# ndpp/ndpp

Hardware: AMD Instinct MI355X
Metric: E_in points*Legendre-orders/sec (free-gas scatter moments) (higher is better)
Workload: dtype f64

## Files before the change

### ndpp_amd/csrc/fg_pipeline.h

```cpp
#pragma once

#include "ndpp_math.h"

namespace ndpp {
#if NDPP_FAST
inline namespace fast_arith {
#else
inline namespace strict_arith {
#endif

#if NDPP_FAST
constexpr int kMuBlock = 2;
#else
constexpr int kMuBlock = 1;
#endif
constexpr int kSegPerGroup = 5;
constexpr int kMaxLevels = 32;
constexpr int kStackLdsLevels = 8;
constexpr int kMaxRows = 2;
constexpr int kSplitLog2 = 4;
constexpr int kSplit = 1 << kSplitLog2;
constexpr int kRowBits = 16;

enum { kStatKEvals = 0, kStatMuVisits, kStatMuIntegrals, kStatEoutNodes,
       kStatWaveIters, kStatLaneIters, kStatOrderVisits, kStatGaussIntegrals, kNumStats };

NDPP_HD unsigned chan_bit(int r, int l) { return 1u << (r * kRowBits + l); }

struct FgBatch {
  int n_jobs, R, G, L, M;
  double A, kT;
  const double* job_A = nullptr;
  const double* job_kT = nullptr;
  const double* job_ein;
  const int* job_row;
  const double* f_tab;
  const double* e_bins;
  double sab_threshold, brent_thresh, mu_tol, eout_tol;
  int mu_its, eout_its;
  MuGrid grid;
  int ncap;
  double* node_a;
  double* node_b;
  double* node_F;
  double* node_S;
  int* node_info;
  int tcap;
  double* t_mulo;
  double* t_muhi;
  double* t_X;
  unsigned char* t_gl = nullptr;
  double gl_ratio = 2.0;
  int gl_near = 1;
  double gl_amin = 2.0E-6;
  int gl_cert_depth = 7;
  int gl_cert_depth_near = 8;
  int gl_panels = 16;
  int gl_graded = 8;
  int* lvl_cnt;
  int* next_task;
  int* overflow;
  unsigned long long* stats;
  double* seg = nullptr;
  int split_below = 0;
  const int* order = nullptr;
  const int* mask_rank = nullptr;
  const int* mu_nodes = nullptr;
  double* raw;

  NDPP_HD double A_of(int job) const { return job_A ? job_A[job] : A; }
  NDPP_HD double kT_of(int job) const { return job_kT ? job_kT[job] : kT; }
  NDPP_HD int nch() const { return R * L; }
  NDPP_HD int n_trees() const { return n_jobs * G * kSegPerGroup; }
  NDPP_HD int lvl_off(int level) const {
    int o = 0;
    for (int k = 0; k < level; ++k) o += lvl_cnt[k];
    return o;
  }
  NDPP_HD bool split_level(int level) const {
    const int nt = n_mu_tasks(level);
    return seg != nullptr && nt > 0 && nt <= split_below;
  }
  NDPP_HD int tasks_per_node(int level) const { return level == 0 ? 5 : 2; }
  NDPP_HD int n_tasks(int level) const { return lvl_cnt[level] * tasks_per_node(level); }
  NDPP_HD int n_mu_tasks(int level) const {
    return (mu_nodes ? *mu_nodes : lvl_cnt[level]) * tasks_per_node(level);
  }
  NDPP_HD int rec_index(int level, int base, int n, int slot) const {
    return level == 0 ? 5 * n + slot : 2 * (n - base) + (slot == 3 ? 1 : 0);
  }
  NDPP_HD double& F(int slot, int ch, int n) const {
    return node_F[((size_t)(slot * R * L + ch)) * ncap + n];
  }
  NDPP_HD double& S(int ch, int n) const { return node_S[(size_t)ch * ncap + n]; }
  NDPP_HD double& tX(int k, int r, int t) const { return t_X[((size_t)(k * R + r)) * tcap + t]; }
  NDPP_HD unsigned full_mask() const {
    unsigned m = 0;
    for (int r = 0; r < R; ++r) m |= ((1u << L) - 1u) << (r * kRowBits);
    return m;
  }
  NDPP_HD int node_job(int n) const { return node_info[4 * n + 2] & 0x3ffffff; }
  NDPP_HD int node_depth(int n) const { return node_info[4 * n + 2] >> 26; }
};

NDPP_HD void fg_setup_group(const FgBatch& B, int job, int g) {
  const double Ein = B.job_ein[job];
  const double A = B.A_of(job), kT = B.kT_of(job);
  double alphaEin = (A - 1.0) / (A + 1.0);
  alphaEin = alphaEin * alphaEin * Ein;
  double Eout_lo, Eout_hi;
  fg_eout_bounds(A, kT, Ein, Eout_lo, Eout_hi);
  const double eg = B.e_bins[g], eg1 = B.e_bins[g + 1];

  double sa[kSegPerGroup], sb[kSegPerGroup];
  bool on[kSegPerGroup] = {false, false, false, false, false};
  if ((eg < Eout_hi) && (eg1 > Eout_lo)) {
    double Elo = (Eout_lo > eg) ? Eout_lo : eg;
    double Ehi = (Eout_hi < eg1) ? Eout_hi : eg1;
    double Ebottom = (eg == 0.0) ? 0.01 * Elo : eg;
    sa[0] = Ebottom; sb[0] = Elo; on[0] = true;
    sa[1] = Ehi;     sb[1] = eg1; on[1] = true;
    if ((Elo < alphaEin) && (alphaEin < Ehi)) {
      sa[2] = Elo; sb[2] = alphaEin; on[2] = true;
      Elo = alphaEin;
    }
    if ((Elo < Ein) && (Ein < Ehi)) {
      sa[3] = Elo; sb[3] = Ein; on[3] = true;
      Elo = Ein;
    }
    sa[4] = Elo; sb[4] = Ehi; on[4] = true;
  } else {
    sa[4] = eg; sb[4] = eg1; on[4] = true;
  }
  const unsigned full = B.full_mask();
  const int nch = B.nch();
  for (int s = 0; s < kSegPerGroup; ++s) {
    int n = (job * B.G + g) * kSegPerGroup + s;
    bool live = on[s] && (sa[s] != sb[s]);
    B.node_a[n] = live ? sa[s] : 0.0;
    B.node_b[n] = live ? sb[s] : 0.0;
    B.node_info[4 * n + 0] = live ? (int)full : 0;
    B.node_info[4 * n + 1] = -1;
    B.node_info[4 * n + 2] = job;
    B.node_info[4 * n + 3] = 0;
    for (int ch = 0; ch < nch; ++ch) B.S(ch, n) = 0.0;
  }
}

NDPP_HD void fg_task_decode(const FgBatch& B, int level, int base, int t, int& n,
                            int& slot) {
  (void)B;
  int idx;
  if (level == 0) {
    idx = t / 5;
    slot = t - 5 * idx;
  } else {
    idx = t >> 1;
    slot = 1 + 2 * (t & 1);
  }
  n = B.order ? B.order[idx] : (level == 0 ? idx : base + idx);
}

NDPP_HD unsigned fg_sort_key(const FgBatch& B, unsigned mask) {
  unsigned m = 0;
  for (int r = 0; r < B.R; ++r) m |= (mask >> (r * kRowBits)) & ((1u << B.L) - 1u);
  return m;
}

constexpr int kSortClasses = 4;
NDPP_HD int fg_node_bucket(const FgBatch& B, int level, int base, int n, int nb) {
  const unsigned mask = (unsigned)B.node_info[4 * n + 0];
  const int last = kSortClasses * nb - 1;
  if (mask == 0) return last;
  double wmax = -1.0;
  const int nslots = B.tasks_per_node(level);
  for (int k = 0; k < nslots; ++k) {
    const int slot = level == 0 ? k : 1 + 2 * k;
    const int rec = B.rec_index(level, base, n, slot);
    unsigned m = mask;
    if (B.t_gl) {
      const unsigned rows = B.t_gl[rec];
      for (int r = 0; r < B.R; ++r)
        if (rows >> r & 1u) m &= ~(((1u << kRowBits) - 1u) << (r * kRowBits));
    }
    if (m == 0) continue;
    const double km = fmax(fmax(fabs(B.tX(0, 0, rec)), fabs(B.tX(1, 0, rec))), fabs(B.tX(2, 0, rec)));
    const double w = (B.t_muhi[rec] - B.t_mulo[rec]) * km;
    wmax = fmax(wmax, w >= 0.0 ? w : 0.0);
  }
  if (wmax < 0.0) return last;
  const int cls = wmax >= 1073741824.0 ? 0 : wmax >= 1048576.0 ? 1 : wmax >= 256.0 ? 2 : 3;
  int b = cls * nb + B.mask_rank[fg_sort_key(B, mask)];
  return b < last ? b : last - 1;
}

NDPP_HD double fg_slot_point(double a, double b, int slot) {
  double c = 0.5 * (a + b);
  switch (slot) {
    case 0: return a;
    case 1: return 0.5 * (a + c);
    case 2: return c;
    case 3: return 0.5 * (c + b);
    default: return b;
  }
}

template <int R>
NDPP_HD void fg_Krows(const FgPair& q, const MuGrid& g, const double* const* f, double mu,
                      double* K) {
#if NDPP_FAST
  const double E = fg_E(q, mu);
#pragma unroll
  for (int r = 0; r < R; ++r) K[r] = (q.C1 * fg_fval(g, f[r], mu)) * E;
#else
  fg_K_rows<R>(q, g, f, mu, K);
#endif
}
NDPP_HD double simpson(double w, double f0, double f1, double f2) {
  return w * (fma(4.0, f1, f0) + f2);
}

NDPP_HD bool fg_gauss_box(int mu_its, double mu_tol) {
  return mu_its >= 15 && mu_tol <= 1.0E-7;
}
constexpr unsigned kGaussNear = 0x80u;
NDPP_HD unsigned fg_gauss_zone(const FgBatch& B, const FgPair& q, double Ein, double Eout) {
  const double amin = (q.EpE - 2.0 * q.s2) / q.AkT;
  if (!(amin >= B.gl_amin)) return 0u;
  const unsigned rows = (1u << B.R) - 1u;
  if (Eout >= B.gl_ratio * Ein || Ein >= B.gl_ratio * Eout) return rows;
  return B.gl_near ? (rows | kGaussNear) : 0u;
}

NDPP_HD void fg_prep_task(const FgBatch& B, int level, int base, int t) {
  int n, slot;
  if (level == 0) { n = t / 5; slot = t - 5 * n; }
  else { n = base + (t >> 1); slot = 1 + 2 * (t & 1); }
  if (B.node_info[4 * n + 0] == 0) {
    if (B.t_gl) B.t_gl[t] = 0;
    return;
  }
  const int job = B.node_job(n);
  const double Ein = B.job_ein[job];
  const double Eout = fg_slot_point(B.node_a[n], B.node_b[n], slot);
  const double A = B.A_of(job);
  const FgPair q = make_pair(A, B.kT_of(job), Ein, Eout);
  double mlo, mhi;
  fg_find_mu(q, A, Ein, Eout, B.sab_threshold, B.brent_thresh, mlo, mhi);
  const double mc = (mlo + mhi) * 0.5;
  B.t_mulo[t] = mlo;
  B.t_muhi[t] = mhi;
  if (B.t_gl) B.t_gl[t] = (unsigned char)fg_gauss_zone(B, q, Ein, Eout);
  for (int r = 0; r < B.R; ++r) {
    const double* fr[1] = {B.f_tab + (size_t)B.job_row[(size_t)job * B.R + r] * B.M};
    fg_Krows<1>(q, B.grid, fr, mlo, &B.tX(0, r, t));
    fg_Krows<1>(q, B.grid, fr, mhi, &B.tX(1, r, t));
    fg_Krows<1>(q, B.grid, fr, mc, &B.tX(2, r, t));
  }
}

#if NDPP_FAST
constexpr int kGaussN = 16;
NDPP_HD double gauss_node(int j) {
  constexpr double x[kGaussN] = {
      -0.98940093499164994, -0.9445750230732326, -0.86563120238783176, -0.755404408355003,
      -0.61787624440264377, -0.45801677765722737, -0.28160355077925892, -0.095012509837637454,
      0.095012509837637454, 0.28160355077925892, 0.45801677765722737, 0.61787624440264377,
      0.755404408355003, 0.86563120238783176, 0.9445750230732326, 0.98940093499164994};
  return x[j];
}
NDPP_HD double gauss_weight(int j) {
  constexpr double w[kGaussN] = {
      0.027152459411754037, 0.062253523938647706, 0.095158511682492591, 0.12462897125553403,
      0.14959598881657676, 0.16915651939500262, 0.18260341504492361, 0.18945061045506859,
      0.18945061045506859, 0.18260341504492361, 0.16915651939500262, 0.14959598881657676,
      0.12462897125553403, 0.095158511682492591, 0.062253523938647706, 0.027152459411754037};
  return w[j];
}

template <int R, int LMAX, bool kAdd = false>
NDPP_HD void gauss_composite(const FgBatch& B, const FgPair& q, const FView<R>& fv, double a, double b,
                             int panels, const PnConsts& pk, double* acc) {
  if (!kAdd) {
#pragma unroll
    for (int ch = 0; ch < R * LMAX; ++ch) acc[ch] = 0.0;
  }
  const double h = (b - a) / (double)(2 * panels);
  for (int p = 0; p < panels; ++p) {
    const double c = a + h * (double)(2 * p + 1);
    for (int j = 0; j < kGaussN; j += 2) {
      const double mu0 = fma(h, gauss_node(j), c), mu1 = fma(h, gauss_node(j + 1), c);
      FvLoad v0[R], v1[R];
      fg_fval_load_rows<R>(B.grid, fv, mu0, v0);
      fg_fval_load_rows<R>(B.grid, fv, mu1, v1);
      double E0, E1;
      fg_E2(q, mu0, mu1, E0, E1);
      E0 *= h * gauss_weight(j);
      E1 *= h * gauss_weight(j + 1);
      double P0[LMAX], P1[LMAX];
      pn_all<LMAX>(mu0, P0, pk);
      pn_all<LMAX>(mu1, P1, pk);
#pragma unroll
      for (int r = 0; r < R; ++r) {
        const double K0 = (q.C1 * fg_fval_use(v0[r])) * E0;
        const double K1 = (q.C1 * fg_fval_use(v1[r])) * E1;
#pragma unroll
        for (int l = 0; l < LMAX; ++l) acc[r * LMAX + l] = fma(K1, P1[l], fma(K0, P0[l], acc[r * LMAX + l]));
      }
    }
  }
}

template <int R, int LMAX>
NDPP_HD void gauss_graded(const FgBatch& B, const FgPair& q, const FView<R>& fv, double a, double b,
                          int m, int split, const PnConsts& pk, double* acc) {
#pragma unroll
  for (int ch = 0; ch < R * LMAX; ++ch) acc[ch] = 0.0;
  const double W = b - a;
  double lo = a;
  for (int k = 1; k <= m + 1; ++k) {
    const double hi = k <= m ? b - ldexp(W, -k) : b;
    gauss_composite<R, LMAX, true>(B, q, fv, lo, hi, split, pk, acc);
// ... 38 lines not shown
    for (int j = 0; j < nn; ++j) {
      const double xa = a + hd * (double)j;
      const double xb = (j == nn - 1) ? b : a + hd * (double)(j + 1);
      const double xc = 0.5 * (xa + xb), xd = 0.5 * (xa + xc), xe = 0.5 * (xc + xb);
      double Kd[R], Ke[R], Kc[R], Kb[R];
      Kat(xd, xe, Kd, Ke);
      if (dep == 0) {
#pragma unroll
        for (int r = 0; r < R; ++r) { Kc[r] = B.tX(2, r, t); Kb[r] = B.tX(1, r, t); }
        evals += 2;
      } else {
        Kat(xc, xb, Kc, Kb);
        if (j == nn - 1) {
#pragma unroll
          for (int r = 0; r < R; ++r) Kb[r] = B.tX(1, r, t);
        }
        evals += 4;
      }
      double Pd[LMAX], Pc[LMAX], Pe[LMAX], Pb[LMAX];
      pn_all<LMAX>(xd, Pd, pk); pn_all<LMAX>(xc, Pc, pk); pn_all<LMAX>(xe, Pe, pk); pn_all<LMAX>(xb, Pb, pk);
      unsigned leaf = 0, big = 0;
#pragma unroll
      for (int r = 0; r < R; ++r) {
        const double Xc2 = 2.0 * Kc[r], Xc4 = 4.0 * Kc[r], Kd4 = 4.0 * Kd[r], Ke4 = 4.0 * Ke[r];
#pragma unroll
        for (int l = 0; l < LMAX; ++l) {
          const double T = fma(Kb[r], Pb[l], Ka[r] * Pa[l]);
          const double s1 = fma(Xc4, Pc[l], T);
          const double s2 = fma(Ke4, Pe[l], fma(Kd4, Pd[l], fma(Xc2, Pc[l], T)));
          const double dS = fabs(fma(w, s2, -(wp * s1)));
          if (mask & chan_bit(r, l)) {
            if (!(dS > eps15)) leaf |= chan_bit(r, l);
            if (dS > big15) big |= chan_bit(r, l);
          }
        }
      }
      const unsigned bad = strict ? leaf : ((leaf & prev_big) | (prev_leaf & big));
#pragma unroll
      for (int r = 0; r < R; ++r)
        if (bad & (((1u << kRowBits) - 1u) << (r * kRowBits))) rows &= ~(1u << r);
      if (rows == 0) return 0;
      prev_leaf = leaf;
      prev_big = big;
#pragma unroll
      for (int r = 0; r < R; ++r) Ka[r] = Kb[r];
#pragma unroll
      for (int l = 0; l < LMAX; ++l) Pa[l] = Pb[l];
    }
  }
  return rows;
}

constexpr int kGaussCertPhases = 2;
constexpr int kGaussPhGraded = kGaussCertPhases;
constexpr int kGaussPhLadder = kGaussCertPhases + 1;
constexpr int kGaussPhases = kGaussCertPhases + 2;
NDPP_HD int gauss_cert_split(int p) {
  return p == 0 ? 0 : p == 1 ? kCertDepth : kMaxLevels;
}

constexpr int kGaussDone = 2;
static_assert(kMaxRows <= kGaussDone, "rows in play and rows done share one byte with kGaussNear");
struct GaussCand {
  int t;
  unsigned st;
};

NDPP_HD int gauss_cert_depth(const FgBatch& B, unsigned st) {
  return (st & kGaussNear) ? B.gl_cert_depth_near : B.gl_cert_depth;
}
NDPP_HD bool gauss_phase_on(const FgBatch& B, int p, unsigned st) {
  if (p < kGaussCertPhases) return gauss_cert_split(p) < gauss_cert_depth(B, st);
  if (p == kGaussPhGraded) return (st & kGaussNear) && B.gl_graded > 0;
  return p == kGaussPhLadder;
}
NDPP_HD int gauss_next_phase(const FgBatch& B, int p, unsigned st) {
  do ++p; while (p < kGaussPhases && !gauss_phase_on(B, p, st));
  return p;
}

template <int R>
NDPP_HD unsigned mu_gauss_entry(const FgBatch& B, int level, int base, int t) {
  unsigned rows = B.t_gl[t];
  if (!rows) return 0;
  const unsigned near = rows & kGaussNear;
  rows &= ~kGaussNear;
  const int n_node = level == 0 ? t / 5 : base + (t >> 1);
  const unsigned mask = (unsigned)B.node_info[4 * n_node + 0];
#pragma unroll
  for (int r = 0; r < R; ++r)
    if (!(mask & (((1u << kRowBits) - 1u) << (r * kRowBits)))) rows &= ~(1u << r);
  if (rows == 0) { B.t_gl[t] = 0; return 0; }
  return rows | near;
}

template <int R, int LMAX>
NDPP_HD int mu_gauss_phase(const FgBatch& B, int level, int base, int p, GaussCand& c, int& next) {
  const int t = c.t;
  const unsigned near = c.st & kGaussNear;
  unsigned rows = c.st & ((1u << R) - 1u);
  unsigned done = (c.st >> kGaussDone) & ((1u << R) - 1u);
  int n_node, slot;
  if (level == 0) { n_node = t / 5; slot = t - 5 * n_node; }
  else { n_node = base + (t >> 1); slot = 1 + 2 * (t & 1); }
  const unsigned mask = (unsigned)B.node_info[4 * n_node + 0];
  const int job = B.node_job(n_node);
  const double Ein = B.job_ein[job];
  const double Eout = fg_slot_point(B.node_a[n_node], B.node_b[n_node], slot);
  const FgPair q = make_pair(B.A_of(job), B.kT_of(job), Ein, Eout);
  FRows f;
  f.off = 8u * (unsigned)B.M * (unsigned)B.job_row[(size_t)job * R];
  const FView<R> fv = f_view<R>(B.f_tab, f, B.M);
  const double a = B.t_mulo[t], b = B.t_muhi[t];
  const PnConsts pk = make_pn_consts();
  int evals = 0;
  auto finish = [&](unsigned taken) {
    B.t_gl[t] = (unsigned char)taken;
    next = kGaussPhases;
  };
  if (p < kGaussCertPhases) {
    const int cd = gauss_cert_depth(B, c.st);
    const int hi = gauss_cert_split(p + 1) < cd ? gauss_cert_split(p + 1) : cd;
    rows = mu_gauss_certify<R, LMAX>(B, q, fv, t, mask, rows, gauss_cert_split(p), hi, pk, evals);
    if (rows == 0) { finish(0u); return evals; }
    c.st = near | rows;
    next = gauss_next_phase(B, p, c.st);
    return evals;
  }
  double Ic[R * LMAX], If[R * LMAX];
  auto take_agreeing_rows = [&]() {
#pragma unroll
    for (int r = 0; r < R; ++r) {
      if (!((rows & ~done) >> r & 1u)) continue;
      bool ok = true;
#pragma unroll
      for (int l = 0; l < LMAX; ++l)
        ok = ok && (fabs(If[r * LMAX + l] - Ic[r * LMAX + l]) <= kGaussAgree * fabs(If[r * LMAX]));
      if (!ok) continue;
      done |= 1u << r;
#pragma unroll
      for (int l = 0; l < LMAX; ++l)
        if (l < B.L && (mask & chan_bit(r, l))) B.F(slot, r * B.L + l, n_node) = If[r * LMAX + l];
    }
  };
  if (p == kGaussPhGraded) {
    gauss_graded<R, LMAX>(B, q, fv, a, b, B.gl_graded, 1, pk, Ic);
    gauss_graded<R, LMAX>(B, q, fv, a, b, B.gl_graded, 2, pk, If);
    evals += 3 * (B.gl_graded + 1) * kGaussN;
    take_agreeing_rows();
    if (done == rows) { finish(rows); return evals; }
    c.st = near | rows | (done << kGaussDone);
    next = kGaussPhLadder;
    return evals;
  }
  gauss_composite<R, LMAX>(B, q, fv, a, b, 4, pk, Ic);
  evals += 4 * kGaussN;
  for (int n = 8;; n *= 2) {
    gauss_composite<R, LMAX>(B, q, fv, a, b, n, pk, If);
    evals += n * kGaussN;
    take_agreeing_rows();
    if (done == rows || 2 * n > B.gl_panels) break;
#pragma unroll
    for (int k = 0; k < R * LMAX; ++k) Ic[k] = If[k];
  }
  finish(done);
  return evals;
}
// ... 321 lines not shown
#pragma unroll
    for (int r = 0; r < R; ++r) { s.Xb[r] = Xbj[r]; s.Xc[r] = Xej[r]; }
    s.wp = wj;
    s.mask = mj;
    s.depth = dj + 1;
    return true;
  }
  return false;
}

template <int R, int LMAX>
NDPP_HD void mu_finish(const FgBatch& B, const MuLane<R, LMAX>& s, bool split = false) {
  const unsigned mask = s.chans;
#pragma unroll
  for (int r = 0; r < R; ++r)
#pragma unroll
    for (int l = 0; l < LMAX; ++l)
      if (mask & chan_bit(r, l)) {
        if (split) {
          if (!s.own_pending)
            B.seg[((size_t)s.task * kSplit + s.slot_path) * B.nch() + r * B.L + l] = s.acc[r * LMAX + l];
          continue;
        }
        B.F(s.slot, r * B.L + l, s.node) = s.tot[r * LMAX + l] + s.acc[r * LMAX + l];
      }
}

template <int R, int LMAX>
NDPP_HD void mu_init_split(const FgBatch& B, int level, int base, int t, MuLane<R, LMAX>& s) {
  const int nt = B.n_mu_tasks(level);
  const int i = t % nt, rank = t / nt;
  mu_init<R, LMAX>(B, level, base, i, s);
  int jp = 0;
  if (s.mask != 0) {
#if NDPP_FAST
    const double pa = s.q.p, qa = s.q.q;
#else
    const double pa = s.q.EpE / s.q.AkT, qa = 2.0 * s.q.s2 / s.q.AkT;
#endif
    const double x = ((pa - fabs(s.q.beta)) / qa - s.a) / (s.b - s.a) * (double)kSplit;
    jp = (x > 0.0) ? (x < (double)(kSplit - 1) ? (int)x : kSplit - 1) : 0;
  }
  int lo = jp - 1, hi = jp, cur = hi;
  for (int k = 0; k <= rank; ++k) {
    if (((k & 1) == 0 && hi < kSplit) || lo < 0) cur = hi++;
    else cur = lo--;
  }
  s.path_left = kSplitLog2;
  s.path_bits = (unsigned)cur;
  s.slot_path = 0;
  int tz = 0;
  while (tz < kSplitLog2 && !(((unsigned)cur >> tz) & 1u)) ++tz;
  s.own_from = kSplitLog2 - tz;
  s.own_pending = (s.own_from != 0);
}

NDPP_HD void fg_mu_combine_task(const FgBatch& B, int level, int base, int t) {
  int n, slot;
  fg_task_decode(B, level, base, t, n, slot);
  const unsigned mask = (unsigned)B.node_info[4 * n + 0];
  if (mask == 0) return;
  const unsigned gl_rows = B.t_gl ? B.t_gl[B.rec_index(level, base, n, slot)] : 0u;
  const int nch = B.nch();
  for (int r = 0; r < B.R; ++r)
    for (int l = 0; l < B.L; ++l)
      if ((mask & chan_bit(r, l)) && !(gl_rows >> r & 1u)) {
        const int ch = r * B.L + l;
        double tot = 0.0;
        for (int j = 0; j < kSplit; ++j) tot = tot + B.seg[((size_t)t * kSplit + j) * nch + ch];
        B.F(slot, ch, n) = tot;
      }
}

struct HostAtomics {
  static int add(int* p, int v) { int o = *p; *p += v; return o; }
};

template <class Atomics>
NDPP_HD void fg_node_process(const FgBatch& B, int level, int base, int i) {
  const int n = base + i;
  const unsigned mask = (unsigned)B.node_info[4 * n + 0];
  if (mask == 0) return;
  const int depth = B.node_depth(n);
  const double a = B.node_a[n], b = B.node_b[n];
  const double c = 0.5 * (a + b);
  const double h = b - a;
  const double w = h / 12.0;
  const double eps15 = 15.0 * ldexp(B.eout_tol, -depth);
  const bool bottom = (B.eout_its - depth) <= 0;
  unsigned refine = 0;
  auto half = [w](double f0, double f1, double f2) { return w * (f0 + 4.0 * f1 + f2); };
  for (int r = 0; r < B.R; ++r)
    for (int l = 0; l < B.L; ++l) {
      if (!(mask & chan_bit(r, l))) continue;
      const int ch = r * B.L + l;
      const double Fa = B.F(0, ch, n), Fd = B.F(1, ch, n), Fc = B.F(2, ch, n),
                   Fe = B.F(3, ch, n), Fb = B.F(4, ch, n);
      double S = B.S(ch, n);
      if (depth == 0) S = (h / 6.0) * (Fa + 4.0 * Fc + Fb);
      const double S2 = half(Fa, Fd, Fc) + half(Fc, Fe, Fb);
      if (bottom || (fabs(S2 - S) <= eps15)) {
        B.S(ch, n) = S2 + (S2 - S) / 15.0;
      } else {
        refine |= chan_bit(r, l);
      }
    }
  B.node_info[4 * n + 3] = (int)refine;
  if (!refine) return;
  const int pos = Atomics::add(&B.lvl_cnt[level + 1], 2);
  const int left = base + B.lvl_cnt[level] + pos;
  if (left + 2 > B.ncap) {
    *B.overflow = 1;
    B.node_info[4 * n + 3] = 0;
    return;
  }
  B.node_info[4 * n + 1] = left;
  const int job = B.node_job(n);
  for (int k = 0; k < 2; ++k) {
    const int m = left + k;
    B.node_a[m] = k ? c : a;
    B.node_b[m] = k ? b : c;
    B.node_info[4 * m + 0] = (int)refine;
    B.node_info[4 * m + 1] = -1;
    B.node_info[4 * m + 2] = job | ((depth + 1) << 26);
    B.node_info[4 * m + 3] = 0;
    for (int r = 0; r < B.R; ++r)
      for (int l = 0; l < B.L; ++l) {
        if (!(refine & chan_bit(r, l))) continue;
        const int ch = r * B.L + l;
        const double f0 = B.F(k ? 2 : 0, ch, n), f1 = B.F(k ? 3 : 1, ch, n), f2 = B.F(k ? 4 : 2, ch, n);
        B.F(0, ch, m) = f0;
        B.F(2, ch, m) = f1;
        B.F(4, ch, m) = f2;
        B.S(ch, m) = half(f0, f1, f2);
      }
  }
}

NDPP_HD void fg_reduce_node(const FgBatch& B, int base, int i) {
  const int n = base + i;
  const unsigned refine = (unsigned)B.node_info[4 * n + 3];
  if (!refine) return;
  const int left = B.node_info[4 * n + 1];
  for (int r = 0; r < B.R; ++r)
    for (int l = 0; l < B.L; ++l)
      if (refine & chan_bit(r, l)) {
        const int ch = r * B.L + l;
        B.S(ch, n) = B.S(ch, left) + B.S(ch, left + 1);
      }
}

NDPP_HD void fg_assemble_call(const FgBatch& B, int call) {
  const int L = B.L, G = B.G;
  const int job = call / B.R, r = call - job * B.R;
  double* out = B.raw + (size_t)call * G * L;
  double p0 = 0.0;
  for (int g = 0; g < G; ++g) {
    const int root = (job * G + g) * kSegPerGroup;
    for (int l = 0; l < L; ++l) {
      const int ch = r * L + l;
      double v = B.S(ch, root + 0) + B.S(ch, root + 1);
      v = v + B.S(ch, root + 2);
      v = v + B.S(ch, root + 3);
      v = v + B.S(ch, root + 4);
      out[g * L + l] = v;
    }
// ... 10 lines not shown
```

### ndpp_amd/csrc/ndpp_hip.hip

```cpp
#include <hip/hip_runtime.h>

#include <algorithm>
#include <chrono>
#include <cmath>
#include <cstdarg>
#include <cstdio>
#include <cstdlib>
#include <cstring>
#include <mutex>
#include <thread>
#include <vector>

#include "../../include/ndpp_hip.h"
#include "dev_util.h"
#include "fg_device.h"
#include "fg_pipeline.h"
#include "kernels.h"

using namespace ndpp;

namespace {

constexpr int kSortMaxMasks = kSortClasses << 11;

// ... 349 lines not shown
  const int NE = (int)edata[1 + 2 * NR];
  if (NE < 1 || 2 + 2 * NR + 2 * NE + 1 > n_edata) return fail(NDPP_EINVAL, "edata: bad NE");
  return NDPP_OK;
}

int ndpp::check_params(const ndpp_params* p, int G, int what, int n_tab) {
  if (!p) return fail(NDPP_EINVAL, "params is NULL");
  if ((what & kCheckOrder) && (p->order < 1 || p->order > NDPP_MAX_ORDER))
    return fail(NDPP_EINVAL, "order=%d outside 1..%d", p->order, NDPP_MAX_ORDER);
  if ((what & kCheckTab) && (n_tab < 1 || n_tab > NDPP_MAX_TAB_BINS))
    return fail(NDPP_EINVAL, "n_tab=%d outside 1..%d", n_tab, NDPP_MAX_TAB_BINS);
  if (p->mu_bins < 2) return fail(NDPP_EINVAL, "mu_bins=%d < 2", p->mu_bins);
  if (G < 1) return fail(NDPP_EINVAL, "need at least one group");
  if (!(what & kCheckFreegas)) return NDPP_OK;
  if (p->adaptive_mu_its < 0 || p->adaptive_mu_its >= kMaxLevels ||
      p->adaptive_eout_its < 0 || p->adaptive_eout_its >= kMaxLevels)
    return fail(NDPP_EINVAL, "adaptive_*_its must be in 0..%d", kMaxLevels - 1);
  const double tols[4] = {p->sab_threshold, p->brent_mu_thresh, p->adaptive_mu_tol, p->adaptive_eout_tol};
  for (double t : tols)
    if (!(t >= 0.0 && t <= 1.7976931348623157e308))
      return fail(NDPP_EINVAL, "tolerances (sab_threshold, brent_mu_thresh, adaptive_*_tol) must be finite and >= 0");
  return NDPP_OK;
}

namespace {

int check_params(const ndpp_params* p, int G) { return ndpp::check_params(p, G, kCheckOrder | kCheckFreegas); }

inline int gs_blocks(long n, int threads = 256) {
  return (int)std::max<long>(1, std::min<long>((n + threads - 1) / threads, 4096));
}

constexpr int kNodesPerCallGuess = 1024;
constexpr int kNumFgContexts = 4;
constexpr int kTwoContextsMinEin = 128;
constexpr int kTwoContextsMaxEin = 15000;
constexpr int kArenaSpareEin = 64;
size_t bytes_per_node(int nch) {
  return sizeof(double) * (2 + 6 * (size_t)nch) + 4 * sizeof(int)
         + 2 * 8 * sizeof(double)
         + 2
         + sizeof(int);
}

struct NucArrays {
  int n_nuc;
  const double *A, *kT, *cutoff, *Q;
  const int* nuc_of_ein;
};

constexpr double kStrictBelowDefault = 0.0;
constexpr double kStrictColdDefault = 1e-4;
constexpr double kStrictRoughDefault = 1e-12;

void arithmetic_switch(int G, double& strict_x, double& strict_cold, double& rough_rho) {
  strict_x = 0.0;
  strict_cold = 0.0;
  rough_rho = -1.0;
#if NDPP_FAST
  strict_x = kStrictBelowDefault;
  if (const char* sx = getenv("NDPP_HIP_STRICT_BELOW")) {
    strict_x = atof(sx);
    if (!(strict_x > 0.0)) { strict_x = 0.0; return; }
  }
  strict_cold = kStrictColdDefault;
  if (const char* sc = getenv("NDPP_HIP_STRICT_COLD")) strict_cold = atof(sc);
  if (G > 2)
    if (const char* sm = getenv("NDPP_HIP_STRICT_MANY")) strict_cold = atof(sm);
  if (!(strict_cold > 0.0)) strict_cold = 0.0;
  rough_rho = kStrictRoughDefault;
  if (const char* sr = getenv("NDPP_HIP_STRICT_ROUGH")) rough_rho = atof(sr);
#else
  (void)G;
#endif
}

struct FgTunables {
  double strict_x, strict_cold, rough_rho;
  bool joint = true;
  long nodes_per_call = 0;
  long max_chunk_ein = 0;
  bool split = true;
  double split_x = 32.0;
  bool gauss = true;
  bool gauss_phased = true;
  bool sort = true;
  long two_min = kTwoContextsMinEin, two_max = kTwoContextsMaxEin;
  double gl_ratio, gl_amin;
  int gl_near, gl_cert_depth, gl_cert_depth_near, gl_graded, gl_panels;
};

FgTunables read_fg_tunables(int G) {
  FgTunables t;
  arithmetic_switch(G, t.strict_x, t.strict_cold, t.rough_rho);
  auto first_is = [](const char* name, char c) { const char* v = getenv(name); return v && v[0] == c; };
  const char* e;
  t.joint = !first_is("NDPP_HIP_NO_JOINT", '1');
  if ((e = getenv("NDPP_HIP_NODES_PER_CALL")) && atol(e) > 0) t.nodes_per_call = atol(e);
  if ((e = getenv("NDPP_HIP_MAX_CHUNK_EIN")) && atol(e) > 0) t.max_chunk_ein = atol(e);
  t.split = !first_is("NDPP_HIP_NO_SPLIT", '1');
  if ((e = getenv("NDPP_HIP_SPLIT_BELOW_X"))) t.split_x = atof(e);
  t.gauss = !first_is("NDPP_HIP_GAUSS", '0');
  t.gauss_phased = !first_is("NDPP_HIP_GAUSS_PHASED", '0');
  t.sort = !first_is("NDPP_HIP_NO_SORT", '1');
  if ((e = getenv("NDPP_HIP_TWO_CONTEXTS_MIN"))) t.two_min = atol(e);
  if ((e = getenv("NDPP_HIP_TWO_CONTEXTS_MAX"))) t.two_max = atol(e);
  const FgBatch d{};
  t.gl_ratio = (e = getenv("NDPP_HIP_GAUSS_RATIO")) ? atof(e) : d.gl_ratio;
  t.gl_near = (e = getenv("NDPP_HIP_GAUSS_NEAR")) ? atoi(e) != 0 : d.gl_near;
  t.gl_amin = (e = getenv("NDPP_HIP_GAUSS_AMIN")) ? atof(e) : d.gl_amin;
  t.gl_cert_depth = (e = getenv("NDPP_HIP_GAUSS_DEPTH")) ? std::min(std::max(atoi(e), 0), 10) : d.gl_cert_depth;
  t.gl_cert_depth_near =
      (e = getenv("NDPP_HIP_GAUSS_DEPTH_NEAR")) ? std::min(std::max(atoi(e), 0), 10) : d.gl_cert_depth_near;
  t.gl_graded = (e = getenv("NDPP_HIP_GAUSS_GRADED")) ? std::min(std::max(atoi(e), 0), 20) : d.gl_graded;
  t.gl_panels = (e = getenv("NDPP_HIP_GAUSS_PANELS")) ? std::min(std::max(atoi(e), 8), 1024) : d.gl_panels;
  return t;
}

struct BatchPlan {
  int joint, nch;
  int num_cu, mu_blocks, split_below;
  int nb_sort;
  size_t mu_threads, seg_doubles, gstack_doubles, ctx_fixed, fixed, need;
  size_t nodes_per_ein;
  long ncap;
  long max_jobs;
  long spare_ein;
  int contexts;
};

int plan_batch(const ndpp_params* p, int n_ein, int n_rows, int G, int rows_per_ein, const FgTunables& t,
               Workspace& g_ws, BatchPlan& pl) {
  const int L = p->order, GL = G * L;
  size_t free_b = 0, total_b = 0;
  pl.joint = (rows_per_ein == 2 && L <= kJointMaxL && t.joint) ? 1 : 0;
  pl.nch = (pl.joint ? 2 : 1) * L;
  pl.nb_sort = kSortClasses << L;
  const size_t per_call_tree = (size_t)G * kSegPerGroup;
  const size_t guess = t.nodes_per_call > 0 ? (size_t)t.nodes_per_call : (size_t)kNodesPerCallGuess;
  pl.contexts = 2;
  pl.spare_ein = t.nodes_per_call > 0 ? 0 : kArenaSpareEin;
  const size_t per_call = std::max<size_t>(guess, 3 * per_call_tree);
  pl.nodes_per_ein = pl.joint ? std::max<size_t>((guess * 5) / 4, 3 * per_call_tree) : per_call * rows_per_ein;
  if (g_ws.num_cu == 0) {
    hipDeviceProp_t prop;
    int dev = 0;
    NDPP_TRY(hipGetDevice(&dev));
    NDPP_TRY(hipGetDeviceProperties(&prop, dev));
    g_ws.num_cu = prop.multiProcessorCount;
  }
  pl.num_cu = g_ws.num_cu;
  pl.mu_blocks = g_ws.num_cu * kMuBlocksPerCU;
  pl.mu_threads = (size_t)pl.mu_blocks * kWave;
  if (pl.mu_threads * DevMuStack<2>::kRecBytes >= ((size_t)1 << 24))
    return fail(NDPP_EDEVICE, "%d compute units: the sibling-stack addressing assumes fewer than 4681 workgroups", g_ws.num_cu);
  pl.gstack_doubles = 0;
  for (int R = 1; R <= (pl.joint ? 2 : 1); ++R) {
    const size_t lv = (size_t)std::max(0, p->adaptive_mu_its - (R == 1 ? mu_lds_levels(1) : mu_lds_levels(2)));
    pl.gstack_doubles = std::max(pl.gstack_doubles, lv * ((R == 1 ? mu_stack_fields(1) : mu_stack_fields(2)) + 1) * pl.mu_threads);
  }
  const size_t split_cap = std::min<size_t>((size_t)1 << 22, std::max<size_t>((size_t)n_ein * 128, (size_t)1 << 16));
  pl.split_below = t.split ? (int)std::min<size_t>((size_t)(t.split_x * pl.mu_threads), split_cap) : 0;
  pl.seg_doubles = (size_t)pl.split_below * kSplit * pl.nch;
  pl.ctx_fixed = (pl.seg_doubles + pl.gstack_doubles + 3) * sizeof(double) +
                 sizeof(int) * (((size_t)kSortClasses << L) + 4 * (kMaxLevels + 2) + 128) + 10 * 256;
  pl.fixed = (size_t)n_ein * 3 * sizeof(int) + (size_t)n_rows * sizeof(int) + (1u << 20) +
             sizeof(int) * ((size_t)1 << L) + pl.contexts * pl.ctx_fixed + 4096;
  const size_t node_bytes = bytes_per_node(pl.nch);
  const size_t whole = pl.fixed + ((size_t)n_ein + pl.contexts * pl.spare_ein) * pl.nodes_per_ein * node_bytes +
                       (size_t)n_ein * rows_per_ein * (sizeof(double) * (GL + 3) + sizeof(int) * 2 + 16) + 4096;
  size_t budget;
  if (g_ws.base && whole <= g_ws.bytes) {
    budget = g_ws.bytes;
    free_b = g_ws.bytes;
  } else {
    NDPP_TRY(hipMemGetInfo(&free_b, &total_b));
    if (g_ws.base) free_b += g_ws.bytes;
    budget = std::min<size_t>((size_t)(free_b * 0.6), (size_t)128 << 30);
  }
  const size_t per_job_bytes = sizeof(double) * (GL + 3) + sizeof(int) * 2 + 16;
  size_t ncap = (budget > pl.fixed ? budget - pl.fixed : 0) /
                (node_bytes + (per_job_bytes * rows_per_ein + pl.nodes_per_ein - 1) / pl.nodes_per_ein);
  ncap = std::min<size_t>(ncap, ((size_t)n_ein + pl.contexts * pl.spare_ein) * pl.nodes_per_ein);
  ncap = std::min<size_t>(ncap, (size_t)0x7fffffff / 5);
  if (t.max_chunk_ein) ncap = std::min<size_t>(ncap, (size_t)t.max_chunk_ein * pl.nodes_per_ein);
  if (ncap < pl.nodes_per_ein)
    return fail(NDPP_ENOMEM, "not enough device memory for one incoming energy (free %zu)", free_b);
  pl.ncap = (long)ncap;
  pl.max_jobs = (long)std::min<size_t>((size_t)n_ein, ncap / pl.nodes_per_ein) * rows_per_ein;
  pl.need = pl.fixed + (size_t)pl.ncap * node_bytes + (size_t)pl.max_jobs * per_job_bytes;
  return NDPP_OK;
}

struct Event {
  hipEvent_t e = nullptr;
  Event() = default;
  Event(Event&& o) noexcept : e(o.e) { o.e = nullptr; }
  ~Event() { if (e) (void)hipEventDestroy(e); }
  hipError_t record(hipStream_t s) {
    const hipError_t rc = e ? hipSuccess : hipEventCreate(&e);
    return rc == hipSuccess ? hipEventRecord(e, s) : rc;
  }
};
struct EventPair { Event before, after; };

struct BatchCall {
  const ndpp_params* p;
  double A, kT, cutoff;
  int n_ein, n_rows, G, rows_per_ein;
  const double *ein, *w_hi, *f_tab, *e_bins;
  const int* row_lo;
  double* out;
  hipStream_t stream;
  NucArrays nuc;
  int GL() const { return G * p->order; }
};

struct Slot {
  int *lvl_cnt, *next_task, *overflow, *mask_hist, *mu_nodes;
  double *seg, *gstack;
  hipStream_t s;
};

struct BatchHead {
  int *fg_list, *f4_list, *fgs_list;
  int* rough;
  int* counters;
  unsigned long long* dstats;
  int* mask_rank;
  Slot slot[kNumFgContexts];
  int n_fast = 0, n_f4 = 0, n_strict = 0;
  BatchHead(Carver& cv, const BatchCall& a, const BatchPlan& pl) {
    fg_list = cv.take<int>(a.n_ein);
    f4_list = cv.take<int>(a.n_ein);
    fgs_list = cv.take<int>(a.n_ein);
    rough = cv.take<int>(a.n_rows);
    counters = cv.take<int>(64);
    dstats = cv.take<unsigned long long>(kNumStats);
    mask_rank = cv.take<int>((size_t)1 << a.p->order);
    for (int k = 0; k < pl.contexts; ++k) {
      Slot& sl = slot[k];
      sl.lvl_cnt = cv.take<int>(kMaxLevels + 2);
      sl.next_task = cv.take<int>(2 * (kMaxLevels + 2));
      sl.overflow = cv.take<int>(64);
      sl.mu_nodes = cv.take<int>(64);
      sl.mask_hist = cv.take<int>(pl.nb_sort);
      sl.seg = cv.take<double>(pl.seg_doubles + 1);
      sl.gstack = cv.take<double>(pl.gstack_doubles + 1);
      sl.s = a.stream;
    }
  }
};

hipError_t upload_mask_rank(int* dst, int nb, hipStream_t stream) {
  std::vector<int> idx(nb), rank(nb);
  for (int m = 0; m < nb; ++m) idx[m] = m;
  std::stable_sort(idx.begin(), idx.end(), [](int x, int y) {
    return __builtin_popcount((unsigned)x) > __builtin_popcount((unsigned)y);
  });
  for (int k = 0; k < nb; ++k) rank[idx[k]] = k;
  hipError_t e = hipMemcpyAsync(dst, rank.data(), sizeof(int) * nb, hipMemcpyHostToDevice, stream);
  if (e != hipSuccess) return e;
  return hipStreamSynchronize(stream);
// ... 41 lines not shown
struct FgCtx {
  FgBatch B;
  Slot sl;
  bool strict;
  const FgStages* stages;
  const int* list;
  int lstride;
  long n, done, chunk_ein, this_ein;
  double *job_ein, *job_A, *job_kT;
  int *job_row, *order;
  bool inflight;
  std::vector<EventPair> walk_ev;
  std::vector<EventPair> gauss_ev;
};

std::vector<FgCtx> deal_contexts(const BatchHead& h, const FgTunables& t, const BatchPlan& pl, bool& side_by_side) {
  std::vector<FgCtx> ctx;
  auto add = [&](const int* list, int parts, long len, bool strict) {
    for (int j = 0; j < parts; ++j) {
      FgCtx c{};
      c.list = list + j; c.lstride = parts; c.n = (len - j + parts - 1) / parts; c.strict = strict;
      c.stages = strict ? &fg_strict_stages() : &kFgOwnStages;
      if (c.n > 0) ctx.push_back(std::move(c));
    }
  };
  auto parts_of = [&](long len, int room) {
    if (len <= 0) return 0;
    const int k = (t.two_min > 0 && len >= t.two_min && len < t.two_max && len >= room) ? room : 1;
    return std::max(1, k);
  };
  const int k_strict = parts_of(h.n_strict, h.n_fast > 0 ? std::max(1, pl.contexts / 2) : pl.contexts);
  const int k_fast = parts_of(h.n_fast, std::max(1, pl.contexts - k_strict));
  add(h.fg_list, k_fast, h.n_fast, false);
  add(h.fgs_list, k_strict, h.n_strict, true);
  const int nctx = (int)ctx.size();
  side_by_side = nctx > 1 && nctx <= pl.contexts && t.two_min > 0 && (size_t)pl.ncap >= (size_t)nctx * pl.nodes_per_ein;
  return ctx;
}

int carve_contexts(std::vector<FgCtx>& ctx, bool side_by_side, const BatchCall& a, const FgTunables& t,
                   const BatchPlan& pl, const BatchHead& h, Carver cv, bool gauss_on, Workspace& ws) {
  const int nctx = (int)ctx.size(), ncap = (int)pl.ncap, L = a.p->order;
  for (int k = 1; side_by_side && k < nctx; ++k)
    if (!ws.aux[k - 1]) NDPP_TRY(hipStreamCreateWithFlags(&ws.aux[k - 1], hipStreamNonBlocking));
  FgBatch T;
  T.gl_ratio = t.gl_ratio; T.gl_near = t.gl_near; T.gl_amin = t.gl_amin; T.gl_cert_depth = t.gl_cert_depth;
  T.gl_cert_depth_near = t.gl_cert_depth_near; T.gl_graded = t.gl_graded; T.gl_panels = t.gl_panels;
  T.G = a.G; T.L = L; T.M = a.p->mu_bins; T.A = a.A; T.kT = a.kT; T.f_tab = a.f_tab; T.e_bins = a.e_bins;
  T.sab_threshold = a.p->sab_threshold; T.brent_thresh = a.p->brent_mu_thresh;
  T.mu_tol = a.p->adaptive_mu_tol; T.eout_tol = a.p->adaptive_eout_tol;
  T.mu_its = a.p->adaptive_mu_its; T.eout_its = a.p->adaptive_eout_its;
  T.grid = make_mu_grid(T.M);
  T.R = pl.joint ? a.rows_per_ein : 1;
  T.mask_rank = h.mask_rank; T.split_below = pl.split_below; T.stats = h.dstats;
  long n_all = 0;
  for (auto& c : ctx) n_all += c.n;
  char* const arena = cv.p;
  long cap_left = ncap;
  for (int k = 0; k < nctx; ++k) {
    FgCtx& c = ctx[k];
    if (!side_by_side) cv.p = arena;
    c.sl = h.slot[side_by_side ? k : 0];
    if (side_by_side && k > 0) c.sl.s = ws.aux[k - 1];
    long share = side_by_side ? std::max<long>((long)pl.nodes_per_ein,
                                               (long)((double)ncap * (c.n + pl.spare_ein) /
                                                      (n_all + (long)nctx * pl.spare_ein))) : ncap;
    share = std::min<long>(share, (long)((size_t)(c.n + pl.spare_ein) * pl.nodes_per_ein));
    if (side_by_side) {
      share = std::min(share, cap_left - (long)(nctx - 1 - k) * (long)pl.nodes_per_ein);
      cap_left -= share;
    }
    const long max_jobs = std::min<long>(c.n, share / (long)pl.nodes_per_ein) * a.rows_per_ein;
    FgBatch& B = c.B;
    B = T;
    B.ncap = (int)share;
    B.node_a = cv.take<double>(B.ncap); B.node_b = cv.take<double>(B.ncap);
    B.node_F = cv.take<double>((size_t)5 * pl.nch * B.ncap);
    B.node_S = cv.take<double>((size_t)pl.nch * B.ncap);
    B.node_info = cv.take<int>((size_t)4 * B.ncap);
    B.tcap = 2 * B.ncap;
    B.t_mulo = cv.take<double>(B.tcap); B.t_muhi = cv.take<double>(B.tcap);
    B.t_X = cv.take<double>((size_t)3 * (pl.joint ? 2 : 1) * B.tcap);
    B.t_gl = (gauss_on && !c.strict) ? cv.take<unsigned char>(B.tcap) : nullptr;
    B.job_ein = c.job_ein = cv.take<double>(max_jobs);
    B.job_row = c.job_row = cv.take<int>(max_jobs);
    c.job_A = cv.take<double>(max_jobs); c.job_kT = cv.take<double>(max_jobs);
    if (a.nuc.nuc_of_ein) { B.job_A = c.job_A; B.job_kT = c.job_kT; }
    B.raw = cv.take<double>((size_t)max_jobs * a.GL());
    c.order = cv.take<int>(B.ncap);
    B.order = t.sort ? c.order : nullptr;
    B.seg = pl.split_below ? c.sl.seg : nullptr;
    B.lvl_cnt = c.sl.lvl_cnt; B.next_task = c.sl.next_task; B.overflow = c.sl.overflow;
    if (cv.p > cv.end)
      return fail(NDPP_ENOMEM, "workspace carve overran (%zu > %zu)",
                  (size_t)(cv.p - ws.base), ws.bytes);
    c.chunk_ein = std::max<long>(1, max_jobs / a.rows_per_ein);
    if (t.max_chunk_ein) c.chunk_ein = std::min<long>(c.chunk_ein, t.max_chunk_ein);
  }
  return NDPP_OK;
}

struct Drain {
  hipStream_t first;
  hipStream_t* more;
  int n_more;
  ~Drain() {
    (void)hipStreamSynchronize(first);
    for (int k = 0; k < n_more; ++k) (void)hipStreamSynchronize(more[k]);
  }
};

struct FgTiming {
  Event ev0, ev1;
  Event ev_f4;
  std::vector<std::pair<float, float>> spans;
  double mu_sum_ms = 0.0, gauss_sum_ms = 0.0;
  double level_ms[32] = {0};
  int mu_launches = 0;

  void fold(std::vector<EventPair>& pairs, bool walk) {
    int level = 0;
    for (auto& e : pairs) {
      float t0 = 0.f, t1 = 0.f;
      if (hipEventElapsedTime(&t0, ev0.e, e.before.e) == hipSuccess &&
          hipEventElapsedTime(&t1, ev0.e, e.after.e) == hipSuccess) {
        (walk ? mu_sum_ms : gauss_sum_ms) += t1 - t0;
        if (walk && level < 32) level_ms[level] += t1 - t0;
        spans.emplace_back(t0, t1);
      }
      ++level;
      if (walk) ++mu_launches;
    }
    pairs.clear();
  }

  void publish(const unsigned long long* hs, int contexts, ndpp_stats* stats) {
    double mu_ms = 0.0;
    std::sort(spans.begin(), spans.end());
    float end = -1.f;
    for (auto& sp : spans) {
      if (sp.second <= end) continue;
      mu_ms += sp.second - std::max(sp.first, end);
      end = sp.second;
    }
    float ms = 0.f, ms4 = 0.f;
    if (hipEventElapsedTime(&ms, ev0.e, ev1.e) == hipSuccess) ndpp::g_last_gpu_ms = ms;
    if (hipEventElapsedTime(&ms4, ev0.e, ev_f4.e) == hipSuccess) {
      profile_add(kProfFile4, ms4);
      profile_add(kProfFreegasMu, mu_ms);
      profile_add(kProfFreegasOther, std::max(0.0, (double)ms - ms4 - mu_ms));
    }
    if (!stats) return;
    stats->k_evals = hs[kStatKEvals];
    stats->mu_visits = hs[kStatMuVisits];
    stats->mu_integrals = hs[kStatMuIntegrals];
    stats->eout_nodes = hs[kStatEoutNodes];
    stats->wave_iters = hs[kStatWaveIters];
    stats->lane_iters = hs[kStatLaneIters];
    stats->order_visits = hs[kStatOrderVisits];
    stats->gauss_integrals = hs[kStatGaussIntegrals];
    stats->gauss_ms = gauss_sum_ms;
    for (int k = 0; k < 32; ++k) stats->mu_level_ms[k] = level_ms[k];
    stats->mu_kernel_ms = mu_sum_ms;
    stats->mu_busy_ms = mu_ms;
    stats->mu_kernel_launches = mu_launches;
    stats->contexts = contexts;
// ... 476 lines not shown
```

Baseline: 302,000.

## Alias shared segment endpoints to reuse adjacent slot integrals

Adds an alias table that links each level-0 segment's left endpoint to the right endpoint of the preceding live segment, across groups, when the two energies are bit-identical. Aliased tasks skip the mu-bound search and Gauss work in prep, and the root integration copies the already computed F values from the source node. This removes duplicate integrals at shared boundaries, at the cost of re-running the group layout for earlier groups during setup and extra workspace per job, which reduces node capacity.

Measured after the change: 305,500 (median of 6 runs). +1.1%, better.

```diff
diff --git a/ndpp_amd/csrc/fg_pipeline.h b/ndpp_amd/csrc/fg_pipeline.h
--- a/ndpp_amd/csrc/fg_pipeline.h
+++ b/ndpp_amd/csrc/fg_pipeline.h
@@ -67,6 +67,7 @@
   const int* mask_rank = nullptr;
   const int* mu_nodes = nullptr;
   double* raw;
+  int* t_alias = nullptr;
 
   NDPP_HD double A_of(int job) const { return job_A ? job_A[job] : A; }
   NDPP_HD double kT_of(int job) const { return job_kT ? job_kT[job] : kT; }
@@ -99,11 +100,12 @@
     for (int r = 0; r < R; ++r) m |= ((1u << L) - 1u) << (r * kRowBits);
     return m;
   }
+  NDPP_HD int alias_of(int level, int rec) const { return (level == 0 && t_alias && t_gl) ? t_alias[rec] : -1; }
   NDPP_HD int node_job(int n) const { return node_info[4 * n + 2] & 0x3ffffff; }
   NDPP_HD int node_depth(int n) const { return node_info[4 * n + 2] >> 26; }
 };
 
-NDPP_HD void fg_setup_group(const FgBatch& B, int job, int g) {
+NDPP_HD void fg_group_layout(const FgBatch& B, int job, int g, double* sa, double* sb, bool* live) {
   const double Ein = B.job_ein[job];
   const double A = B.A_of(job), kT = B.kT_of(job);
   double alphaEin = (A - 1.0) / (A + 1.0);
@@ -112,7 +114,6 @@
   fg_eout_bounds(A, kT, Ein, Eout_lo, Eout_hi);
   const double eg = B.e_bins[g], eg1 = B.e_bins[g + 1];
 
-  double sa[kSegPerGroup], sb[kSegPerGroup];
   bool on[kSegPerGroup] = {false, false, false, false, false};
   if ((eg < Eout_hi) && (eg1 > Eout_lo)) {
     double Elo = (Eout_lo > eg) ? Eout_lo : eg;
@@ -132,18 +133,58 @@
   } else {
     sa[4] = eg; sb[4] = eg1; on[4] = true;
   }
+  for (int s = 0; s < kSegPerGroup; ++s) live[s] = on[s] && (sa[s] != sb[s]);
+}
+NDPP_HD int fg_chain_slot(int k) {
+  constexpr int chain[kSegPerGroup] = {0, 2, 3, 4, 1};
+  return chain[k];
+}
+
+NDPP_HD bool same_bits(double x, double y) {
+#if defined(__HIP_DEVICE_COMPILE__)
+  return __double_as_longlong(x) == __double_as_longlong(y);
+#else
+  long long a, b;
+  __builtin_memcpy(&a, &x, sizeof a);
+  __builtin_memcpy(&b, &y, sizeof b);
+  return a == b;
+#endif
+}
+
+NDPP_HD void fg_setup_group(const FgBatch& B, int job, int g) {
+  double sa[kSegPerGroup], sb[kSegPerGroup];
+  bool live[kSegPerGroup];
+  fg_group_layout(B, job, g, sa, sb, live);
   const unsigned full = B.full_mask();
   const int nch = B.nch();
   for (int s = 0; s < kSegPerGroup; ++s) {
     int n = (job * B.G + g) * kSegPerGroup + s;
-    bool live = on[s] && (sa[s] != sb[s]);
-    B.node_a[n] = live ? sa[s] : 0.0;
-    B.node_b[n] = live ? sb[s] : 0.0;
-    B.node_info[4 * n + 0] = live ? (int)full : 0;
+    B.node_a[n] = live[s] ? sa[s] : 0.0;
+    B.node_b[n] = live[s] ? sb[s] : 0.0;
+    B.node_info[4 * n + 0] = live[s] ? (int)full : 0;
     B.node_info[4 * n + 1] = -1;
     B.node_info[4 * n + 2] = job;
     B.node_info[4 * n + 3] = 0;
     for (int ch = 0; ch < nch; ++ch) B.S(ch, n) = 0.0;
+  }
+  if (!B.t_alias) return;
+  const int root = (job * B.G + g) * kSegPerGroup;
+  for (int k = 0; k < 5 * kSegPerGroup; ++k) B.t_alias[5 * root + k] = -1;
+  int prev = -1;
+  double prev_b = 0.0;
+  for (int gp = g - 1; gp >= 0 && prev < 0; --gp) {
+    double pa[kSegPerGroup], pb[kSegPerGroup];
+    bool pl[kSegPerGroup];
+    fg_group_layout(B, job, gp, pa, pb, pl);
+    for (int k = 0; k < kSegPerGroup; ++k)
+      if (pl[fg_chain_slot(k)]) { prev = root - (g - gp) * kSegPerGroup + fg_chain_slot(k); prev_b = pb[fg_chain_slot(k)]; }
+  }
+  for (int k = 0; k < kSegPerGroup; ++k) {
+    const int s = fg_chain_slot(k);
+    if (!live[s]) continue;
+    if (prev >= 0 && same_bits(prev_b, sa[s])) B.t_alias[5 * (root + s) + 0] = 5 * prev + 4;
+    prev = root + s;
+    prev_b = sb[s];
   }
 }
 
@@ -224,6 +265,7 @@
   return mu_its >= 15 && mu_tol <= 1.0E-7;
 }
 constexpr unsigned kGaussNear = 0x80u;
+constexpr unsigned kGaussAlias = 0x40u;
 NDPP_HD unsigned fg_gauss_zone(const FgBatch& B, const FgPair& q, double Ein, double Eout) {
   const double amin = (q.EpE - 2.0 * q.s2) / q.AkT;
   if (!(amin >= B.gl_amin)) return 0u;
@@ -238,6 +280,10 @@
   else { n = base + (t >> 1); slot = 1 + 2 * (t & 1); }
   if (B.node_info[4 * n + 0] == 0) {
     if (B.t_gl) B.t_gl[t] = 0;
+    return;
+  }
+  if (B.alias_of(level, t) >= 0) {
+    B.t_gl[t] = (unsigned char)(kGaussAlias | ((1u << B.R) - 1u));
     return;
   }
   const int job = B.node_job(n);
@@ -442,7 +488,7 @@
 template <int R>
 NDPP_HD unsigned mu_gauss_entry(const FgBatch& B, int level, int base, int t) {
   unsigned rows = B.t_gl[t];
-  if (!rows) return 0;
+  if (!rows || (rows & kGaussAlias)) return 0;
   const unsigned near = rows & kGaussNear;
   rows &= ~kGaussNear;
   const int n_node = level == 0 ? t / 5 : base + (t >> 1);
@@ -930,6 +976,15 @@
   const unsigned mask = (unsigned)B.node_info[4 * n + 0];
   if (mask == 0) return;
   const int depth = B.node_depth(n);
+  if (level == 0 && B.t_alias) {
+    const int src = B.t_alias[5 * n + 0];
+    if (src >= 0) {
+      const int sn = src / 5, ss = src - 5 * sn;
+      for (int r = 0; r < B.R; ++r)
+        for (int l = 0; l < B.L; ++l)
+          if (mask & chan_bit(r, l)) B.F(0, r * B.L + l, n) = B.F(ss, r * B.L + l, sn);
+    }
+  }
   const double a = B.node_a[n], b = B.node_b[n];
   const double c = 0.5 * (a + b);
   const double h = b - a;
diff --git a/ndpp_amd/csrc/ndpp_hip.hip b/ndpp_amd/csrc/ndpp_hip.hip
--- a/ndpp_amd/csrc/ndpp_hip.hip
+++ b/ndpp_amd/csrc/ndpp_hip.hip
@@ -455,6 +455,7 @@
   long max_chunk_ein = 0;
   bool split = true;
   double split_x = 32.0;
+  bool alias = true;
   bool gauss = true;
   bool gauss_phased = true;
   bool sort = true;
@@ -473,6 +474,7 @@
   if ((e = getenv("NDPP_HIP_MAX_CHUNK_EIN")) && atol(e) > 0) t.max_chunk_ein = atol(e);
   t.split = !first_is("NDPP_HIP_NO_SPLIT", '1');
   if ((e = getenv("NDPP_HIP_SPLIT_BELOW_X"))) t.split_x = atof(e);
+  t.alias = !first_is("NDPP_HIP_NO_ALIAS", '1');
   t.gauss = !first_is("NDPP_HIP_GAUSS", '0');
   t.gauss_phased = !first_is("NDPP_HIP_GAUSS_PHASED", '0');
   t.sort = !first_is("NDPP_HIP_NO_SORT", '1');
@@ -540,8 +542,9 @@
   pl.fixed = (size_t)n_ein * 3 * sizeof(int) + (size_t)n_rows * sizeof(int) + (1u << 20) +
              sizeof(int) * ((size_t)1 << L) + pl.contexts * pl.ctx_fixed + 4096;
   const size_t node_bytes = bytes_per_node(pl.nch);
+  const size_t per_job_bytes = sizeof(double) * (GL + 3) + sizeof(int) * 2 + 16 + sizeof(int) * 25 * (size_t)G;
   const size_t whole = pl.fixed + ((size_t)n_ein + pl.contexts * pl.spare_ein) * pl.nodes_per_ein * node_bytes +
-                       (size_t)n_ein * rows_per_ein * (sizeof(double) * (GL + 3) + sizeof(int) * 2 + 16) + 4096;
+                       (size_t)n_ein * rows_per_ein * per_job_bytes + 4096;
   size_t budget;
   if (g_ws.base && whole <= g_ws.bytes) {
     budget = g_ws.bytes;
@@ -551,7 +554,6 @@
     if (g_ws.base) free_b += g_ws.bytes;
     budget = std::min<size_t>((size_t)(free_b * 0.6), (size_t)128 << 30);
   }
-  const size_t per_job_bytes = sizeof(double) * (GL + 3) + sizeof(int) * 2 + 16;
   size_t ncap = (budget > pl.fixed ? budget - pl.fixed : 0) /
                 (node_bytes + (per_job_bytes * rows_per_ein + pl.nodes_per_ein - 1) / pl.nodes_per_ein);
   ncap = std::min<size_t>(ncap, ((size_t)n_ein + pl.contexts * pl.spare_ein) * pl.nodes_per_ein);
@@ -759,6 +761,7 @@
     B.t_mulo = cv.take<double>(B.tcap); B.t_muhi = cv.take<double>(B.tcap);
     B.t_X = cv.take<double>((size_t)3 * (pl.joint ? 2 : 1) * B.tcap);
     B.t_gl = (gauss_on && !c.strict) ? cv.take<unsigned char>(B.tcap) : nullptr;
+    B.t_alias = (t.alias && B.t_gl) ? cv.take<int>((size_t)25 * a.G * max_jobs) : nullptr;
     B.job_ein = c.job_ein = cv.take<double>(max_jobs);
     B.job_row = c.job_row = cv.take<int>(max_jobs);
     c.job_A = cv.take<double>(max_jobs); c.job_kT = cv.take<double>(max_jobs);
```
